# CITlabRostock/citlab-article-separation-new

Measured on AMD Instinct MI355X. Metric: newspaper pages/sec (ARU-Net seg + GNN relation) at 3000x4500 px, higher is better.
Workload: dtype f32s

## Files before the change

citlab-article-separation-new_amd/csrc/aru_engine.hip:

```cpp
#include <algorithm>
#include <cmath>
#include <cstdlib>
#include <memory>

#include "aru_kernels.h"
#include "res8_kernels.h"
#include "res8v_kernels.h"
#include "bf16_kernels.h"
#include "res8w_kernels.h"
#include "res8ws_kernels.h"
#include "level0_plan.h"
#include "convr_kernels.h"
#include "split_kernels.h"
#include "asep_common.h"
#include "aru_pack.h"

using namespace asep;

namespace {

struct Tensor {
    float* p = nullptr;
    int H = 0, W = 0, C = 0;
    bool bf = false;
    size_t count() const { return (size_t)H * W * C; }
    bf16_t* bp() const { return reinterpret_cast<bf16_t*>(p); }
};

struct PackedConv : ConvPlan {
    float* d_w = nullptr;
    float* d_b = nullptr;
    float* d_wino = nullptr;
    float* d_wv = nullptr;
    bf16_t* d_wb = nullptr;
    bf16_t* d_wb8 = nullptr;
    bf16_t* d_ws = nullptr;
    bf16_t* d_ws16 = nullptr;
};

struct DirectConv {
    int k = 0, cout = 0;
    float* d_w = nullptr;
    float* d_b = nullptr;
};

}

struct asep_aru {
    asep_aru_cfg cfg{};
    std::map<std::string, PackedConv> convs;
    struct ResB { int C = 0; bf16_t* d_w = nullptr; float* d_b = nullptr; };
    std::map<std::string, ResB> resb;
    bf16_t* d_r8b_down_w = nullptr;
    float* d_r8b_down_b = nullptr;
    bf16_t* d_r8b_up_w1 = nullptr;
    bf16_t* d_r8f_up_w1 = nullptr;
    bf16_t* d_r8f_down_w1 = nullptr;
    float* d_r8b_down_w1r = nullptr;
    bool use_res32 = true;
    int walk_mode = 1;
    bool use_deconvs = true;
    bool use_convr = true;
    unsigned char* d_zero_trash = nullptr;
    int fused_act = 0;
    bool use_walk = true;
    bf16_t* d_r8b_up_w = nullptr;
    float* d_r8b_up_b = nullptr;
    float* d_r8b_up_b1 = nullptr;
    DirectConv det_first, att_first;
    float* d_r8_down_wr = nullptr;
    float* d_r8_down_br = nullptr;
    float* d_r8_up_w1 = nullptr;
    float* d_r8_up_wr = nullptr;
    float* d_r8_up_br = nullptr;
    float* d_r8_up_b1 = nullptr;
    float* d_r8v_down_wr = nullptr;
    float* d_r8v_up_w1 = nullptr;
    float* d_r8v_up_wr = nullptr;
    bool r8_valu = true;
    bool use_split_walk = true;
    bf16_t* d_r8ws_down_w = nullptr;
    bf16_t* d_r8ws_up_w = nullptr;
    bf16_t* d_r8ws_up_w1 = nullptr;
    bool use_fused8 = true;
    bool fused8_wanted = true;
    bool fused8_var = false;
    float* d_att_head = nullptr;
    bf16_t* d_att_headb = nullptr;
    float* d_logit_w = nullptr;
    float* d_logit_b = nullptr;
    float* d_logit_wd = nullptr;
    float* d_stats = nullptr;
    double* d_sums = nullptr;
    struct Lane {
        hipStream_t s = nullptr;
        bool own_stream = false;
        hipStream_t side = nullptr;
        hipEvent_t ev_fork = nullptr, ev_join = nullptr, ev_begin = nullptr, ev_done = nullptr;
        hipStream_t bside = nullptr;
        hipEvent_t ev_bfork = nullptr, ev_bjoin = nullptr;
        BufferPool pool;
        ~Lane() {
            if (ev_fork) (void)hipEventDestroy(ev_fork);
            if (ev_bfork) (void)hipEventDestroy(ev_bfork);
            if (ev_bjoin) (void)hipEventDestroy(ev_bjoin);
            if (ev_join) (void)hipEventDestroy(ev_join);
            if (ev_begin) (void)hipEventDestroy(ev_begin);
            if (ev_done) (void)hipEventDestroy(ev_done);
            if (side) (void)hipStreamDestroy(side);
            if (bside) (void)hipStreamDestroy(bside);
            if (own_stream && s) (void)hipStreamDestroy(s);
        }
    };
    std::vector<std::unique_ptr<Lane>> lanes;
    Lane* cur = nullptr;
    int last_nl = 0;
    bool lanes_forced = false;
    int num_lanes = 2;
    std::map<std::string, Tensor> endpoints;
    hipStream_t stream = nullptr;
    std::vector<void*> owned;

    struct ProfRec { int kid; double flops, bytes, xflops; hipEvent_t a, b; };
    int num_cus = 256;
    BufferPool host_stage;
    hipStream_t host_stream = nullptr;
    bool use_xcd_sched = true;
    std::map<std::string, const int32_t*> sched_cache;
    bool bf16 = false;
    bool split = false;
    bool use_c12 = true;
    bool fuse_pool = true;
    bool fuse_act = true;
    bool profiling = false;
    bool prof_detail = false;
    bool prof_in_situ = false;
    std::vector<std::string> prof_names;
    std::vector<ProfRec> prof_recs;
    std::vector<hipEvent_t> ev_pool;
    size_t ev_next = 0;

    ~asep_aru() {
        for (void* p : owned)
            if (p) (void)hipFree(p);
// ... 100 lines not shown
    return d;
}

const int32_t* tile_schedule(asep_aru* m, const Res8Args& a, int nblocks, int unit_h) {
    if (!m->use_xcd_sched || nblocks % 8 != 0 || a.total_tiles < 2 * nblocks) return nullptr;
    std::vector<TileDims> probs;
    for (int i = 0; i < a.nprob; ++i) probs.push_back({a.p[i].tiles_x, (a.p[i].H + unit_h - 1) / unit_h, a.p[i].tile_begin});
    return xcd_schedule(m, probs, a.total_tiles);
}

XcdMap oneshot_map(asep_aru* m, int total, int* n_units) {
    XcdMap xm{0, total};
    if (n_units) *n_units = total;
    if (!m->use_xcd_sched || total < 8 * 64) return xm;
    xm.chunk = (total + 7) / 8;
    if (n_units) *n_units = 8 * xm.chunk;
    return xm;
}

typedef std::vector<Tensor> TL;

Tensor new_tensor(asep_aru* m, int H, int W, int C) {
    Tensor t;
    t.H = H; t.W = W; t.C = C;
    t.p = (float*)m->cur->pool.get(t.count() * sizeof(float));
    return t;
}

inline double tbytes(const Tensor& t) { return (double)t.count() * (t.bf ? 2.0 : 4.0); }

std::string dims_of(const TL& l) {
    std::string d;
    for (size_t i = 0; i < l.size() && i < 3; ++i) d += (i ? "+" : "") + std::to_string(l[i].H) + "x" + std::to_string(l[i].W);
    if (l.size() > 3) d += "+..(" + std::to_string(l.size()) + ")";
    return d;
}

#define ASEP_CONV_LAUNCH(KH_, KW_, MT_, C8_, TH_, DB_, BF_, C12_, MB_)                                                   \
    do {                                                                                                                 \
        ps.set_name("conv_mfma_kernel" + targs({ti(KH_), ti(KW_), ti(MT_), tb(C8_), ti(TH_), tb(DB_), tb(BF_), tb(C12_), ti(MB_)})); \
        hipLaunchKernelGGL((conv_mfma_kernel<KH_, KW_, MT_, C8_, TH_, DB_, BF_, C12_, MB_>), grid, dim3(256), 0, s, a);  \
    } while (0)

template <int KH, int KW>
void launch_conv_k(asep_aru* m, const PackedConv& pc, const ConvArgs& a, int total_tiles, double flops, double bytes,
                   const std::string& scope, const TL& in0, bool big_tile) {
    const int mt = pc.c8 ? 1 : (pc.mtiles % 4 == 0 ? 4 : (pc.mtiles % 2 == 0 ? 2 : 1));
    dim3 grid(total_tiles, pc.mtiles / mt);
    ProfScope ps(m, "conv_mfma_kernel", flops, scope + " " + dims_of(in0) + " " + std::to_string(pc.cin) + "->" + std::to_string(pc.cout));
    ps.bytes = bytes;
    hipStream_t s = m->stream;
    const bool res_op = a.p[0].res != nullptr;
    const bool has_res = res_op || KH != 3;
    if constexpr (KW == 4) {
        if (pc.c12) {
            ASEP_CONV_LAUNCH(KH, KW, 1, false, 16, false, false, true, 2);
            return;
        }
    }
    if constexpr (KH == 3) {
        if (pc.c8 && big_tile && !res_op) {
            ASEP_CONV_LAUNCH(3, 3, 1, true, 16, false, false, false, 4);
            return;
        }
    }
    if (pc.c8) ASEP_CONV_LAUNCH(KH, KW, 1, true, CONV_TH, true, false, false, 2);
    else if (mt == 1 && big_tile && !has_res) ASEP_CONV_LAUNCH(3, 3, 1, false, 16, false, false, false, 4);
    else if (mt == 1 && big_tile) ASEP_CONV_LAUNCH(KH, KW, 1, false, 16, false, false, false, 2);
    else if (mt == 4) ASEP_CONV_LAUNCH(KH, KW, 4, false, CONV_TH, true, false, false, 2);
    else if (mt == 2 && !res_op) ASEP_CONV_LAUNCH(KH, KW, 2, false, CONV_TH, true, false, false, 3);
    else if (mt == 2) ASEP_CONV_LAUNCH(KH, KW, 2, false, CONV_TH, true, false, false, 2);
    else ASEP_CONV_LAUNCH(KH, KW, 1, false, CONV_TH, true, false, false, 2);
}

enum PoolKind { POOL_MAX, POOL_AVG_C1, POOL_CHANSUM };
TL run_pool(asep_aru* m, const TL& in, PoolKind kind);

#define ASEP_CONVS_LAUNCH(KH_, KW_, C16_, MT_, TH_, MB_)                                                              \
    do {                                                                                                              \
        ps.set_name("convs_kernel" + targs({ti(KH_), ti(KW_), tb(C16_), ti(MT_), ti(TH_), ti(MB_)}));                 \
        hipLaunchKernelGGL((convs_kernel<KH_, KW_, C16_, MT_, TH_, MB_>), grid, dim3(256), 0, m->stream, a);          \
    } while (0)

TL run_conv_split(asep_aru* m, const PackedConv& pc, const std::string& scope, const TL& in0, const TL* in1, bool relu_in, bool relu_out,
                  const TL* res, TL* pooled, bool keep_full, int act) {
    const bool fuse_pool = pooled && m->fuse_pool;
    TL out;
    if (keep_full || !fuse_pool)
        for (const Tensor& t : in0) out.push_back(new_tensor(m, t.H, t.W, pc.cout));
    if (fuse_pool) {
        pooled->clear();
        for (const Tensor& t : in0) pooled->push_back(new_tensor(m, (t.H + 1) / 2, (t.W + 1) / 2, pc.cout));
    }
    const bool c16 = pc.smode == 1;
    const bool alds = pc.d_ws16 && pc.mtiles == 1;
    const int mt = (pc.mtiles % 4 == 0 && !c16) ? 4 : (pc.mtiles % 2 == 0 ? 2 : 1);
    const int th = (c16 && pc.kh == 3 && mt == 1) ? 16 : 8;
    for (size_t b0 = 0; b0 < in0.size(); b0 += MAXP) {
        const size_t b1 = std::min(in0.size(), b0 + MAXP);
        ConvArgs a{};
        int tiles = 0;
        double flops = 0, bytes = (double)pc.kh * pc.kw * pc.cin * pc.cout * 4.0;
        for (size_t i = b0; i < b1; ++i) {
            ConvProb& p = a.p[i - b0];
            p.in0 = in0[i].p; p.in1 = in1 ? (*in1)[i].p : nullptr; p.res = res ? (*res)[i].p : nullptr;
            p.out = out.empty() ? nullptr : out[i].p;
            p.pool = fuse_pool ? (*pooled)[i].p : nullptr;
            p.H = p.Ho = in0[i].H; p.W = p.Wo = in0[i].W;
            p.tiles_x = (in0[i].W + 31) / 32;
            p.tile_begin = tiles;
            tiles += p.tiles_x * ((in0[i].H + th - 1) / th);
            flops += 2.0 * in0[i].H * in0[i].W * pc.kh * pc.kw * (double)pc.cin * pc.cout;
            bytes += tbytes(in0[i]) + (in1 ? tbytes((*in1)[i]) : 0.0) + (res ? tbytes((*res)[i]) : 0.0) + (out.empty() ? 0.0 : tbytes(out[i])) +
                     (fuse_pool ? tbytes((*pooled)[i]) : 0.0);
        }
        a.nprob = (int)(b1 - b0);
        a.total_tiles = tiles;
        a.c0 = in0[0].C; a.c1 = in1 ? (*in1)[0].C : 0;
        a.wpk = (const f32x4*)(alds ? pc.d_ws16 : pc.d_ws); a.bias = pc.d_b;
        a.cout = pc.cout; a.mtiles = pc.mtiles; a.groups = alds ? pc.cin / 16 : pc.cin / 32;
        a.relu_in = relu_in; a.relu_out = relu_out; a.act = act;
        a.skip_full = fuse_pool && !keep_full;
        int units = tiles;
        a.xm = oneshot_map(m, tiles, &units);
        dim3 grid(units, pc.mtiles / mt);
        TL sub(in0.begin() + b0, in0.begin() + b1);
        ProfScope ps(m, "convs_kernel", flops, scope + " " + dims_of(sub) + " " + std::to_string(pc.cin) + "->" + std::to_string(pc.cout));
        ps.bytes = bytes;
        if (alds) {
            ps.set_name("convs16_kernel<1,8,3,true>");
            hipLaunchKernelGGL((convs16_kernel<1, 8, 3, true>), grid, dim3(256), 0, m->stream, a);
        } else if (pc.kh == 3) {
            if (c16 && th == 16) ASEP_CONVS_LAUNCH(3, 3, true, 1, 16, 2);
            else if (c16 && mt == 2) ASEP_CONVS_LAUNCH(3, 3, true, 2, 8, 3);
            else if (c16) ASEP_CONVS_LAUNCH(3, 3, true, 1, 8, 3);
            else if (mt == 4) ASEP_CONVS_LAUNCH(3, 3, false, 4, 8, 2);
            else if (mt == 2) ASEP_CONVS_LAUNCH(3, 3, false, 2, 8, 2);
            else ASEP_CONVS_LAUNCH(3, 3, false, 1, 8, 2);
        } else {
            if (c16 && mt == 2) ASEP_CONVS_LAUNCH(4, 4, true, 2, 8, 2);
            else if (c16) ASEP_CONVS_LAUNCH(4, 4, true, 1, 8, 2);
            else { set_error("internal: conv %s (4x4, %d input channels) was packed for the split-product kernel", scope.c_str(), pc.cin); throw ArgError(); }
        }
    }
    if (pooled && !fuse_pool) *pooled = run_pool(m, out, POOL_MAX);
    return out;
}


TL run_conv(asep_aru* m, const std::string& scope, const TL& in0, const TL* in1, bool relu_in, bool relu_out,
            const TL* res, TL* pooled = nullptr, bool keep_full = true, int act = 0) {
    auto it = m->convs.find(scope);
    if (it == m->convs.end()) { set_error("internal: conv %s not packed", scope.c_str()); throw ArgError(); }
    const PackedConv& pc = it->second;
    const int cin = in0[0].C + (in1 ? (*in1)[0].C : 0);
    if (cin != pc.cin) {
        set_error("internal: conv %s expects Cin=%d, got %d", scope.c_str(), pc.cin, cin);
        throw ArgError();
    }
    if (!((pc.kh == 3 && pc.kw == 3) || (pc.kh == 4 && pc.kw == 4))) {
        set_error("conv %s: unsupported kernel size %dx%d", scope.c_str(), pc.kh, pc.kw);
        throw ArgError();
    }
    if (pc.d_wv && pc.cout == 1 && m->r8_valu && !in1 && !res && !pooled) {
        TL out1;
        for (const Tensor& t : in0) out1.push_back(new_tensor(m, t.H, t.W, 1));
        for (size_t b0 = 0; b0 < in0.size(); b0 += MAXP) {
            const size_t b1 = std::min(in0.size(), b0 + MAXP);
            ConvArgs a{};
            int tiles = 0;
            double flops = 0, bytes = 0;
            for (size_t i = b0; i < b1; ++i) {
                ConvProb& p = a.p[i - b0];
                p.in0 = in0[i].p; p.out = out1[i].p;
                p.H = p.Ho = in0[i].H; p.W = p.Wo = in0[i].W;
                p.tiles_x = cdiv(in0[i].W, C1O_T);
                p.tile_begin = tiles;
                tiles += p.tiles_x * cdiv(in0[i].H, C1O_T);
                flops += 2.0 * in0[i].H * in0[i].W * 16.0 * pc.cin;
                bytes += tbytes(in0[i]) + tbytes(out1[i]);
            }
            a.nprob = (int)(b1 - b0);
            a.total_tiles = tiles;
            a.c0 = pc.cin; a.cout = 1;
            a.wpk = (const f32x4*)pc.d_wv; a.bias = pc.d_b;
            a.relu_in = relu_in; a.relu_out = relu_out; a.act = act;
            int units = tiles;
            a.xm = oneshot_map(m, tiles, &units);
            ProfScope ps(m, "conv_c1out_kernel", flops, scope);
            ps.bytes = bytes;
            hipLaunchKernelGGL(conv_c1out_kernel, dim3(units), dim3(256), 0, m->stream, a);
        }
        return out1;
    }
    if (m->split && pc.d_ws) return run_conv_split(m, pc, scope, in0, in1, relu_in, relu_out, res, pooled, keep_full, act);
    const bool wino = pc.d_wino && pc.mtiles > 1;
    const int wino_mt = pc.mtiles % 4 == 0 ? 4 : (pc.mtiles % 2 == 0 ? 2 : 1);
    const bool fuse_pool = pooled && m->fuse_pool && pc.cout % 4 == 0 && (!wino || wino_mt <= 2);
    TL out;
    if (keep_full || !fuse_pool)
        for (const Tensor& t : in0) out.push_back(new_tensor(m, t.H, t.W, pc.cout));
    if (fuse_pool) {
        pooled->clear();
        for (const Tensor& t : in0) pooled->push_back(new_tensor(m, cdiv(t.H, 2), cdiv(t.W, 2), pc.cout));
    }
    const bool big_tile = !wino && (!pc.c8 || (pc.kh == 3 && !res)) && (pc.groups == 1 || (pc.groups == 2 && !res && pc.kh == 3)) && pc.mtiles == 1;
    const int th = big_tile ? 16 : CONV_TH;
    for (size_t b0 = 0; b0 < in0.size(); b0 += MAXP) {
        const size_t b1 = std::min(in0.size(), b0 + MAXP);
        ConvArgs a{};
        int tiles = 0;
        double flops = 0, bytes = (double)pc.kh * pc.kw * pc.cin * pc.cout * 4.0;
        for (size_t i = b0; i < b1; ++i) {
            ConvProb& p = a.p[i - b0];
            p.in0 = in0[i].p; p.in1 = in1 ? (*in1)[i].p : nullptr; p.res = res ? (*res)[i].p : nullptr;
            p.out = out.empty() ? nullptr : out[i].p;
            p.pool = fuse_pool ? (*pooled)[i].p : nullptr;
            p.H = p.Ho = in0[i].H; p.W = p.Wo = in0[i].W;
// ... 1346 lines not shown
        }
        reserve_lds({(const void*)res8_down_kernel<false>, (const void*)res8v_down_kernel<0>, (const void*)res8v_down_kernel<1>, (const void*)res8v_down_kernel<2>},
                    R8_DOWN_LDS, "residual");
    }
    if (m->split && !variant && m->d_r8_down_wr) {
        const Res8wsPack p = pack_res8ws(blob, up);
        m->d_r8ws_up_w = m->put_some(p.up_w);
        m->d_r8ws_up_w1 = m->put_some(p.up_w1);
        m->d_r8ws_down_w = m->put_some(p.down_w);
    }
    m->fused_act = (m->bf16 && variant && !cfg->plain_u && cfg->activation != 0 && m->fused8_wanted && m->fuse_act) ? cfg->activation : 0;
    const bool fusedb = m->bf16 && (!variant || m->fused_act);
    if (fusedb && cfg->res_depth == 3 && cfg->feat_root == 8) {
        const Res8bPack p = pack_res8b(blob, up);
        m->d_r8b_down_w = m->put_some(p.down_w);
        m->d_r8b_down_b = m->put_some(p.down_b);
        m->d_r8f_down_w1 = m->put_some(p.f_down_w1);
        m->d_r8b_down_w1r = m->put_some(p.down_w1r);
        m->d_r8b_up_w = m->put_some(p.up_w);
        m->d_r8b_up_b = m->put_some(p.up_b);
        m->d_r8b_up_w1 = m->put_some(p.up_w1);
        m->d_r8b_up_b1 = m->put_some(p.up_b1);
        m->d_r8f_up_w1 = m->put_some(p.f_up_w1);
    }
    if (fusedb && cfg->res_depth == 3)
        for (int l = 0; l < n; ++l) {
            const int f = cfg->feat_root << l;
            if (f != 8 && f != 16 && !(f == 32 && m->use_res32)) continue;
            for (const char* side : {"down", "up"}) {
                if (side[0] == 'u' && l == n - 1) continue;
                const std::string scope = std::string("aru_net/featMapG/unet_") + side + "_" + std::to_string(l);
                const ResbPack p = pack_resb(blob, scope, f);
                if (p.ok) m->resb[scope] = {f, m->put(p.w), m->put(p.b)};
            }
        }
    const Layer logit = find_layer(blob, "aru_net/logit/class");
    if (!has_shape(logit.w, 4, 4, cfg->feat_root, cfg->n_classes)) {
        set_error("weights: aru_net/logit/class/weights must be [4,4,%d,%d]", cfg->feat_root, cfg->n_classes);
        throw PackRefusal{ASEP_ERR_WEIGHTS};
    }
    m->d_logit_w = m->put(logit.w.data);
    m->d_logit_b = m->put(logit.b.data);
    if (cfg->n_classes == 2) m->d_logit_wd = m->put(pack_logit_diff(logit));
}

}

extern "C" {

asep_aru* asep_aru_load(const void* weight_blob, size_t nbytes, const asep_aru_cfg* cfg) {
    ASEP_GUARD_BEGIN
    if (!cfg || !weight_blob) { set_error("asep_aru_load: null argument"); return nullptr; }
    if (cfg->struct_size != (int32_t)sizeof(asep_aru_cfg)) {
        set_error("asep_aru_load: cfg.struct_size is %d, this library's asep_aru_cfg has %zu bytes (ABI version %d): the binding was "
                  "written against another include/asep_hip.h", cfg->struct_size, sizeof(asep_aru_cfg), ASEP_ABI_VERSION);
        return nullptr;
    }
    if (cfg->channels != 1) { set_error("asep_aru_load: only 1-channel input is supported (ARU_v1.py:115)"); return nullptr; }
    if (cfg->compute_dtype < 0 || cfg->compute_dtype > 2) { set_error("asep_aru_load: compute_dtype %d unknown (0 = fp32, 1 = bf16 MFMA, 2 = fp32 with split bf16 products)", cfg->compute_dtype); return nullptr; }
    if (cfg->scale_space_num < 1 || cfg->res_depth < 1) { set_error("asep_aru_load: bad cfg"); return nullptr; }
    if (cfg->activation < 0 || cfg->activation > 2) { set_error("asep_aru_load: activation %d unknown (0 = relu, 1 = elu, 2 = leaky)", cfg->activation); return nullptr; }
    const bool variant = cfg->activation != 0 || cfg->plain_u != 0;
    if (cfg->plain_u && cfg->use_attention) { set_error("asep_aru_load: graph 'U' has no attention branch (ARU_v1.py:92-97)"); return nullptr; }
    std::map<std::string, HostTensor> blob;
    if (!parse_blob(weight_blob, nbytes, blob)) return nullptr;
    warn_ignored_switches();
    std::unique_ptr<asep_aru> m(new asep_aru());
    m->cfg = *cfg;
    m->bf16 = cfg->compute_dtype == 1;
    m->split = cfg->compute_dtype == 2;
    if (const char* e = getenv("ASEP_FUSE_POOL")) m->fuse_pool = atoi(e) != 0;
    if (const char* e = getenv("ASEP_FUSE_ACT")) m->fuse_act = atoi(e) != 0;
    if (const char* e = getenv("ASEP_C12")) m->use_c12 = atoi(e) != 0;
    if (const char* e = getenv("ASEP_FUSED8")) m->use_fused8 = atoi(e) != 0;
    m->fused8_wanted = m->use_fused8;
    if (variant) m->use_fused8 = false;
    if (const char* e = getenv("ASEP_R8_VALU")) m->r8_valu = atoi(e) != 0;
    m->fused8_var = variant && !cfg->plain_u && cfg->activation != 0 && m->fused8_wanted && m->r8_valu && m->fuse_act && !m->bf16;
    if (const char* e = getenv("ASEP_XCD_SCHED")) m->use_xcd_sched = atoi(e) != 0;
    if (const char* e = getenv("ASEP_BF_RES32")) m->use_res32 = atoi(e) != 0;
    if (const char* e = getenv("ASEP_BF_CONVR")) m->use_convr = atoi(e) != 0;
    if (const char* e = getenv("ASEP_SPLIT_DECONV")) m->use_deconvs = atoi(e) != 0;
    if (const char* e = getenv("ASEP_SPLIT_WALK")) m->use_split_walk = atoi(e) != 0;
    if (const char* e = getenv("ASEP_BF_WALK")) { m->walk_mode = atoi(e); m->use_walk = m->walk_mode != 0; }
    if (const char* e = getenv("ASEP_LANES")) { m->num_lanes = std::max(1, std::min(4, atoi(e))); m->lanes_forced = true; }
    for (int l = 0; l < m->num_lanes; ++l) {
        std::unique_ptr<asep_aru::Lane> L(new asep_aru::Lane());
        bool ok = hipStreamCreateWithFlags(&L->side, hipStreamNonBlocking) == hipSuccess &&
                  hipStreamCreateWithFlags(&L->bside, hipStreamNonBlocking) == hipSuccess &&
                  hipEventCreateWithFlags(&L->ev_fork, hipEventDisableTiming) == hipSuccess &&
                  hipEventCreateWithFlags(&L->ev_bfork, hipEventDisableTiming) == hipSuccess &&
                  hipEventCreateWithFlags(&L->ev_bjoin, hipEventDisableTiming) == hipSuccess &&
                  hipEventCreateWithFlags(&L->ev_join, hipEventDisableTiming) == hipSuccess &&
                  hipEventCreateWithFlags(&L->ev_begin, hipEventDisableTiming) == hipSuccess &&
                  hipEventCreateWithFlags(&L->ev_done, hipEventDisableTiming) == hipSuccess;
        if (ok && l > 0) { ok = hipStreamCreateWithFlags(&L->s, hipStreamNonBlocking) == hipSuccess; L->own_stream = ok; }
        if (!ok) { set_error("asep_aru_load: cannot create streams/events for lane %d", l); return nullptr; }
        m->lanes.push_back(std::move(L));
    }
    m->cur = m->lanes[0].get();
    try {
        load_weights(m.get(), blob, variant);
    } catch (const PackRefusal&) {
        return nullptr;
    }
    {
        hipDeviceProp_t prop;
        int dev = 0;
        if (hipGetDevice(&dev) == hipSuccess && hipGetDeviceProperties(&prop, dev) == hipSuccess && prop.multiProcessorCount > 0)
            m->num_cus = prop.multiProcessorCount;
    }
    m->d_stats = m->alloc<float>(2);
    m->d_sums = m->alloc<double>(2);
    m->d_zero_trash = m->alloc<unsigned char>(8192);
    ASEP_HIP_CHECK_THROW(hipMemset(m->d_zero_trash, 0, 8192));
    return m.release();
    ASEP_GUARD_END_PTR
}

void asep_aru_free(asep_aru* m) { delete m; }

static int forward_lanes(asep_aru* m, int n_pages, const float* const* d_imgs, const int32_t* Hs, const int32_t* Ws, float* const* d_outs,
                         uint8_t* const* d_u8, uint8_t* const* d_mask, float threshold, hipStream_t stream) {
    m->endpoints.clear();
    const int by_pages = m->lanes_forced ? n_pages : n_pages / 4;
    const int nl = (m->profiling || n_pages < 2) ? 1 : std::max(1, std::min<int>((int)m->lanes.size(), by_pages));
    asep_aru::Lane& L0 = *m->lanes[0];
    L0.s = stream;
    if (nl != m->last_nl && n_pages > 1) {
        if (m->last_nl != 0)
            for (auto& Lp : m->lanes) Lp->pool.release();
        m->last_nl = nl;
    }
    if (nl == 1) return forward_impl(m, L0, 0, n_pages, d_imgs, Hs, Ws, d_outs, d_u8, d_mask, threshold);
    ASEP_HIP_CHECK(hipEventRecord(L0.ev_begin, stream));
    int page0 = 0;
    for (int l = 0; l < nl; ++l) {
        asep_aru::Lane& L = *m->lanes[l];
        const int cnt = n_pages / nl + (l < n_pages % nl ? 1 : 0);
        if (l > 0) ASEP_HIP_CHECK(hipStreamWaitEvent(L.s, L0.ev_begin, 0));
        int rc = forward_impl(m, L, page0, cnt, d_imgs + page0, Hs + page0, Ws + page0, d_outs + page0, d_u8 ? d_u8 + page0 : nullptr,
                              d_mask ? d_mask + page0 : nullptr, threshold);
        if (rc) return rc;
        if (l > 0) {
            ASEP_HIP_CHECK(hipEventRecord(L.ev_done, L.s));
            ASEP_HIP_CHECK(hipStreamWaitEvent(stream, L.ev_done, 0));
        }
        page0 += cnt;
    }
    m->stream = stream;
    return ASEP_OK;
}

int asep_aru_forward_dev(asep_aru* m, const float* d_img, int H, int W, float* d_out, uint8_t* d_out_u8,
                         uint8_t* d_out_mask, float threshold, void* stream) {
    ASEP_GUARD_BEGIN
    if (!m || !d_img || !d_out || H < 1 || W < 1) { set_error("asep_aru_forward_dev: bad argument"); return ASEP_ERR_ARG; }
    const int32_t h1 = H, w1 = W;
    return forward_lanes(m, 1, &d_img, &h1, &w1, &d_out, d_out_u8 ? &d_out_u8 : nullptr, d_out_mask ? &d_out_mask : nullptr,
                         threshold, (hipStream_t)stream);
    ASEP_GUARD_END
}

int asep_aru_forward_batch_dev(asep_aru* m, int n_pages, const float* const* d_imgs, int H, int W, float* const* d_outs,
                               uint8_t* const* d_out_u8, uint8_t* const* d_out_mask, float threshold, void* stream) {
    ASEP_GUARD_BEGIN
// ... 161 lines not shown
```

citlab-article-separation-new_amd/csrc/asep_common.hip:

```cpp
#include "asep_common.h"
#include <cstdlib>

namespace asep {

static thread_local char g_err[1024] = "";

void set_error(const char* fmt, ...) {
    va_list ap;
    va_start(ap, fmt);
    vsnprintf(g_err, sizeof(g_err), fmt, ap);
    va_end(ap);
}
const char* get_error() { return g_err; }

void warn_ignored_switches() {
    static bool done = false;
    if (done) return;
    done = true;
    static const char* const gone[] = {
        "ASEP_F32_SPLIT", "ASEP_SPLIT_L0", "ASEP_SPLIT_ALDS", "ASEP_SPLIT_TH16", "ASEP_WINOGRAD", "ASEP_WINO_REG", "ASEP_WINO16", "ASEP_BIGTILE",
        "ASEP_BIGTILE2", "ASEP_XCD_ONESHOT", "ASEP_SIDE_STREAM", "ASEP_FUSED8_VAR", "ASEP_BF_TH8", "ASEP_BF_MTB", "ASEP_BF_W8", "ASEP_BF_R8B",
        "ASEP_BF_R8F", "ASEP_CONVS_DBG", "ASEP_R8S_DBG", "ASEP_MAXP24",
#ifndef ASEP_ABLATION
        "ASEP_GNN_BATCH", "ASEP_GNN_LANES",
#endif
    };
    for (const char* name : gone)
        if (getenv(name))
            fprintf(stderr, "libasep_hip: %s is set but is not a switch of this build (ignored; asep_engine_switches() lists what is read)\n", name);
}

bool parse_blob(const void* blob, size_t nbytes, std::map<std::string, HostTensor>& out) {
    const uint8_t* p = (const uint8_t*)blob;
    if (!p || nbytes < 12 || memcmp(p, "ASEPW001", 8) != 0) {
        set_error("weight blob: bad magic (expected ASEPW001)");
        return false;
    }
    uint32_t n;
    memcpy(&n, p + 8, 4);
    size_t off = 12;
    for (uint32_t i = 0; i < n; ++i) {
        if (off + 2 > nbytes) { set_error("weight blob: truncated"); return false; }
        uint16_t nl;
        memcpy(&nl, p + off, 2);
        off += 2;
        if (off + nl + 1 > nbytes) { set_error("weight blob: truncated"); return false; }
        std::string name((const char*)p + off, nl);
        off += nl;
        uint8_t nd = p[off];
        off += 1;
        HostTensor t;
        if (off + 4u * nd > nbytes) { set_error("weight blob: truncated"); return false; }
        for (int d = 0; d < nd; ++d) {
            uint32_t v;
            memcpy(&v, p + off, 4);
            off += 4;
            t.dims.push_back((int)v);
        }
        size_t cnt = t.count();
        if (off + 4 * cnt > nbytes) { set_error("weight blob: truncated in %s", name.c_str()); return false; }
        t.data.resize(cnt);
        memcpy(t.data.data(), p + off, 4 * cnt);
        off += 4 * cnt;
        out[name] = std::move(t);
    }
    if (off != nbytes) { set_error("weight blob: %zu trailing bytes", nbytes - off); return false; }
    return true;
}

void* BufferPool::get(size_t bytes) {
    if (bytes == 0) bytes = 16;
    if (next_ < bufs_.size()) {
        Buf& b = bufs_[next_];
        if (b.n < bytes) {
            if (b.p) (void)hipFree(b.p);
            b.p = nullptr;
            b.n = 0;
            ASEP_HIP_CHECK_THROW(hipMalloc(&b.p, bytes));
            b.n = bytes;
        }
        ++next_;
        return b.p;
    }
    Buf b{nullptr, 0};
    ASEP_HIP_CHECK_THROW(hipMalloc(&b.p, bytes));
    b.n = bytes;
    bufs_.push_back(b);
    ++next_;
    return b.p;
}

void BufferPool::release() {
    for (auto& b : bufs_)
        if (b.p) (void)hipFree(b.p);
    bufs_.clear();
    next_ = 0;
}

size_t BufferPool::total_bytes() const {
    size_t t = 0;
    for (auto& b : bufs_) t += b.n;
    return t;
}

}

extern "C" {
// ... 64 lines not shown
```

citlab-article-separation-new_amd/csrc/split_kernels.h:

```cpp
#pragma once
#include "bf16_kernels.h"
#include "res8_kernels.h"

namespace asep {

__device__ __forceinline__ void split3_pair(float a, float b, unsigned& h, unsigned& m, unsigned& l) {
    h = pack_bf16x2(a, b);
    const f32x2 r = psub(f32x2{a, b}, f32x2{__uint_as_float(h << 16), __uint_as_float(h & 0xffff0000u)});
    m = pack_bf16x2(r.x, r.y);
    const f32x2 q = psub(r, f32x2{__uint_as_float(m << 16), __uint_as_float(m & 0xffff0000u)});
    l = pack_bf16x2(q.x, q.y);
}
__device__ __forceinline__ void split3_x8(f32x4 v0, f32x4 v1, u32x4& h, u32x4& m, u32x4& l) {
    unsigned hh[4], mm[4], ll[4];
    split3_pair(v0.x, v0.y, hh[0], mm[0], ll[0]);
    split3_pair(v0.z, v0.w, hh[1], mm[1], ll[1]);
    split3_pair(v1.x, v1.y, hh[2], mm[2], ll[2]);
    split3_pair(v1.z, v1.w, hh[3], mm[3], ll[3]);
    h = u32x4{hh[0], hh[1], hh[2], hh[3]};
    m = u32x4{mm[0], mm[1], mm[2], mm[3]};
    l = u32x4{ll[0], ll[1], ll[2], ll[3]};
}

template <int KH, int KW, bool C16, int MT, int TH, int MINB>
__global__ __launch_bounds__(256, MINB) void convs_kernel(const ConvArgs a) {
    constexpr int TW = 32, NT = TH * 2 / 4, NH = NT > 4 ? NT / 2 : NT;
    static_assert(NT % 4 == 0, "a wave owns whole row pairs (fused 2x2 pool)");
    constexpr int LH = TH + KH - 1, LW = TW + KW - 1;
    constexpr int PT = (KH - 1) / 2, PL = (KW - 1) / 2;
    constexpr int TAPS = KH * KW;
    constexpr int SUBS = C16 ? 2 : 4;
    constexpr int PLANE = LH * LW * 32, NPL = C16 ? 1 : 2, PART = NPL * PLANE;
    constexpr int CPS = C16 ? (TAPS + 1) / 2 : TAPS;
    constexpr int NU = LH * LW * SUBS, NLOAD = (NU + 255) / 256;
    static_assert(3 * PART <= 65536, "halo tile of the three parts in 64 KB");
    __shared__ __attribute__((aligned(16))) unsigned char lds[3 * PART];

    const int tid = threadIdx.x, lane = tid & 63, wave = tid >> 6;
    const int j = lane & 15, kk = lane >> 4;
    const int bid = sched_tile(a.xm);
    if (bid < 0) return;
    int pi = 0;
    pi = prob_of_tile(a, bid);
    const ConvProb& P = a.p[pi];
    const int tile = bid - P.tile_begin;
    const int ty = tile / P.tiles_x, tx = tile - ty * P.tiles_x;
    const int x0 = tx * TW, y0 = ty * TH, mt0 = blockIdx.y * MT;
    const int H = P.H, W = P.W, cout = a.cout;

    f32x4 acc[MT][NT];
#pragma unroll
    for (int m = 0; m < MT; ++m) {
        const int c = (mt0 + m) * 16 + kk * 4;
        const f32x4 b4 = c < cout ? *reinterpret_cast<const f32x4*>(a.bias + c) : f32x4{0.f, 0.f, 0.f, 0.f};
#pragma unroll
        for (int n = 0; n < NT; ++n) acc[m][n] = b4;
    }
    int nbase[NT];
#pragma unroll
    for (int n = 0; n < NT; ++n) {
        const int id = wave * NT + n;
        nbase[n] = ((id >> 1) * LW + (id & 1) * 16 + j) * 32 + (kk & 1) * 16 + (C16 ? 0 : (kk >> 1) * PLANE);
    }
    if (P.res) {
#pragma unroll
        for (int m = 0; m < MT; ++m) {
            const int c = (mt0 + m) * 16 + kk * 4;
            if (c < cout) {
#pragma unroll
                for (int n = 0; n < NT; ++n) {
                    const int id = wave * NT + n;
                    const int y = min(y0 + (id >> 1), H - 1), x = min(x0 + (id & 1) * 16 + j, W - 1);
                    acc[m][n] += *reinterpret_cast<const f32x4*>(P.res + ((size_t)y * W + x) * cout + c);
                }
            }
        }
    }
    const int nchunks = (C16 ? 1 : a.groups) * CPS;
    const u32x4* __restrict__ wsrc = reinterpret_cast<const u32x4*>(a.wpk) + (size_t)mt0 * 64 + lane;
    const size_t wpart = (size_t)a.mtiles * 64;
    u32x4 af[3][MT], afn[3][MT];
    auto fetch = [&](int q, u32x4 (&dst)[3][MT]) {
        const u32x4* __restrict__ s0 = wsrc + (size_t)q * 3 * wpart;
#pragma unroll
        for (int s = 0; s < 3; ++s)
#pragma unroll
            for (int m = 0; m < MT; ++m) dst[s][m] = s0[s * wpart + m * 64];
    };
    fetch(0, af);

    int spix[NLOAD], slds[NLOAD];
    unsigned stmask = 0;
#pragma unroll
    for (int i = 0; i < NLOAD; ++i) {
        const int u = min(tid + i * 256, NU - 1);
        const int pix = u / SUBS, sub = u - pix * SUBS;
        const int ly = pix / LW, lx = pix - ly * LW;
        const int gy = y0 - PT + ly, gx = x0 - PL + lx;
        spix[i] = min(max(gy, 0), H - 1) * W + min(max(gx, 0), W - 1);
        slds[i] = (sub >> 1) * PLANE + pix * 32 + (sub & 1) * 16;
        stmask |= ((gy >= 0 && gy < H && gx >= 0 && gx < W && tid + i * 256 < NU) ? 1u : 0u) << i;
    }
    const int sub0 = (tid % SUBS) * 8;
    const int cin = a.c0 + a.c1;

    int q = 0;
    const int ngroups = C16 ? 1 : a.groups;
    for (int g = 0; g < ngroups; ++g) {
        {
            const int c = g * 32 + sub0;
            const bool from0 = c < a.c0;
            const float* __restrict__ src = concat_src(P.in0, P.in1, c, a.c0);
            const int cs = from0 ? a.c0 : a.c1;
            const bool second = c + 4 < cin;
            f32x4 st0[NLOAD], st1[NLOAD];
#pragma unroll
            for (int i = 0; i < NLOAD; ++i) {
                const float* p = src + (size_t)spix[i] * cs;
                st0[i] = *reinterpret_cast<const f32x4*>(p);
                st1[i] = second ? *reinterpret_cast<const f32x4*>(p + 4) : f32x4{0.f, 0.f, 0.f, 0.f};
            }
            if (g > 0) __syncthreads();
#pragma unroll
            for (int i = 0; i < NLOAD; ++i) {
                if (i * 256 + 255 < NU || tid + i * 256 < NU) {
                    f32x4 v0 = st0[i], v1 = st1[i];
                    if (!((stmask >> i) & 1u)) v0 = v1 = f32x4{0.f, 0.f, 0.f, 0.f};
                    if (a.relu_in) { v0 = relu4(v0); v1 = relu4(v1); }
                    u32x4 h, mm, l;
                    split3_x8(v0, v1, h, mm, l);
                    *reinterpret_cast<u32x4*>(lds + slds[i]) = h;
                    *reinterpret_cast<u32x4*>(lds + PART + slds[i]) = mm;
                    *reinterpret_cast<u32x4*>(lds + 2 * PART + slds[i]) = l;
                }
            }
            __syncthreads();
        }
        auto chunk = [&](int toff) {
            fetch(min(q + 1, nchunks - 1), afn);
            __builtin_amdgcn_sched_barrier(0);
#pragma unroll
            for (int nh = 0; nh < NT; nh += NH) {
                u32x4 bh[NH], bm[NH], bl[NH];
#pragma unroll
                for (int n = 0; n < NH; ++n) {
                    const unsigned char* p = lds + nbase[nh + n] + toff;
                    bh[n] = *reinterpret_cast<const u32x4*>(p);
                    bm[n] = *reinterpret_cast<const u32x4*>(p + PART);
                    bl[n] = *reinterpret_cast<const u32x4*>(p + 2 * PART);
                }
#pragma unroll
                for (int m = 0; m < MT; ++m)
#pragma unroll
                    for (int n = 0; n < NH; ++n) {
                        f32x4 c = acc[m][nh + n];
                        c = mfma_bf16_k32(af[2][m], bh[n], c);
                        c = mfma_bf16_k32(af[0][m], bl[n], c);
                        c = mfma_bf16_k32(af[1][m], bm[n], c);
                        c = mfma_bf16_k32(af[1][m], bh[n], c);
                        c = mfma_bf16_k32(af[0][m], bm[n], c);
                        c = mfma_bf16_k32(af[0][m], bh[n], c);
                        acc[m][nh + n] = c;
                    }
            }
#pragma unroll
            for (int s = 0; s < 3; ++s)
#pragma unroll
                for (int m = 0; m < MT; ++m) af[s][m] = afn[s][m];
            ++q;
        };
        if constexpr (C16) {
#pragma unroll
            for (int t = 0; t < CPS; ++t) {
                const int ta = 2 * t, tb = 2 * t + 1 < TAPS ? 2 * t + 1 : TAPS - 1;
                const int oa = ((ta / KW) * LW + ta % KW) * 32, ob = ((tb / KW) * LW + tb % KW) * 32;
                chunk((kk >> 1) ? ob : oa);
            }
        } else {
#pragma unroll 1
            for (int ky = 0; ky < KH; ++ky)
#pragma unroll
                for (int kx = 0; kx < KW; ++kx) chunk((ky * LW + kx) * 32);
        }
    }

    const int Wp = (W + 1) >> 1;
#pragma unroll
    for (int m = 0; m < MT; ++m) {
        const int c = (mt0 + m) * 16 + kk * 4;
        const bool cok = c < cout;
#pragma unroll
        for (int n = 0; n < NT; ++n) {
            const int id = wave * NT + n;
            const int y = y0 + (id >> 1), x = x0 + (id & 1) * 16 + j;
            const bool ok = cok && y < H && x < W;
            const size_t p = ((size_t)min(y, H - 1) * W + min(x, W - 1)) * cout + (cok ? c : 0);
            f32x4 v = acc[m][n];
            if (a.relu_out) v = relu4(v);
            else if (a.act) v = act4(v, a.act);
            acc[m][n] = v;
            if (ok && !a.skip_full) *reinterpret_cast<f32x4*>(P.out + p) = v;
        }
        if (P.pool) {
#pragma unroll
            for (int n = 0; n < NT; ++n) {
                if (n & 2) continue;
                const int id = wave * NT + n;
                const int y = y0 + (id >> 1), x = x0 + (id & 1) * 16 + j;
                pool2_store(acc[m][n], acc[m][n + 2], y + 1 < H, x + 1 < W, (j & 1) == 0 && cok && y < H && x < W,
                            P.pool + ((size_t)(y >> 1) * Wp + (x >> 1)) * cout + (cok ? c : 0));
            }
        }
    }
}


template <int MT, int TH, int MINB, bool ALDS>
__global__ __launch_bounds__(256, MINB) void convs16_kernel(const ConvArgs a) {
    constexpr int KH = 3, KW = 3, TW = 32, NT = TH * 2 / 4;
    static_assert(NT == 4, "8 x 32 tiles: a wave owns two rows");
    constexpr int LH = TH + KH - 1, LW = TW + KW - 1, PT = 1, PL = 1, TAPS = 9, CPS = 5;
    constexpr int PART = LH * LW * 32;
    constexpr int NU = LH * LW * 2, NLOAD = (NU + 255) / 256;
    constexpr int ABUF = ALDS ? 3 * MT * 1024 : 0;
    __shared__ __attribute__((aligned(16))) unsigned char lds[3 * PART + 2 * ABUF + 16];
    unsigned char* const albs = lds + 3 * PART;

    const int tid = threadIdx.x, lane = tid & 63, wave = tid >> 6;
    const int j = lane & 15, kk = lane >> 4;
    const int bid = sched_tile(a.xm);
    if (bid < 0) return;
    int pi = 0;
    pi = prob_of_tile(a, bid);
    const ConvProb& P = a.p[pi];
    const int tile = bid - P.tile_begin;
    const int ty = tile / P.tiles_x, tx = tile - ty * P.tiles_x;
    const int x0 = tx * TW, y0 = ty * TH, mt0 = blockIdx.y * MT;
    const int H = P.H, W = P.W, cout = a.cout;

    f32x4 acc[MT][NT];
#pragma unroll
    for (int m = 0; m < MT; ++m) {
        const int c = (mt0 + m) * 16 + kk * 4;
        const f32x4 b4 = c < cout ? *reinterpret_cast<const f32x4*>(a.bias + c) : f32x4{0.f, 0.f, 0.f, 0.f};
#pragma unroll
        for (int n = 0; n < NT; ++n) acc[m][n] = b4;
    }
    int nbase[NT];
#pragma unroll
    for (int n = 0; n < NT; ++n) {
        const int id = wave * NT + n;
        nbase[n] = ((id >> 1) * LW + (id & 1) * 16 + j) * 32 + (kk & 1) * 16;
    }
    if (P.res) {
#pragma unroll
        for (int m = 0; m < MT; ++m) {
            const int c = (mt0 + m) * 16 + kk * 4;
            if (c < cout) {
#pragma unroll
                for (int n = 0; n < NT; ++n) {
                    const int id = wave * NT + n;
                    const int y = min(y0 + (id >> 1), H - 1), x = min(x0 + (id & 1) * 16 + j, W - 1);
                    acc[m][n] += *reinterpret_cast<const f32x4*>(P.res + ((size_t)y * W + x) * cout + c);
                }
            }
// ... 303 lines not shown
```

Baseline: 149.7.

## Pipeline next channel-group input loads behind MFMA work in split conv kernel

Adds a PIPE variant of the split-precision 3x3 conv kernel for non-C16 layers with mt 2 or 4. The global loads for channel group g+1 are issued during the first tap's MFMA chunk and written to LDS after the current group finishes, so memory latency hides behind compute. For MT=4 the weight prefetch is interleaved per m-row instead of held in a full double-buffer, which lowers register pressure. The trade-off is more live registers for the staged input, an extra barrier per group, and less freedom for the scheduler.

Result: no change. 150.2 (median of 4 runs) (+0.3%).

```diff
diff --git a/citlab-article-separation-new_amd/csrc/aru_engine.hip b/citlab-article-separation-new_amd/csrc/aru_engine.hip
--- a/citlab-article-separation-new_amd/csrc/aru_engine.hip
+++ b/citlab-article-separation-new_amd/csrc/aru_engine.hip
@@ -60,6 +60,7 @@
     bool use_res32 = true;
     int walk_mode = 1;
     bool use_deconvs = true;
+    bool use_split_pipe = true;
     bool use_convr = true;
     unsigned char* d_zero_trash = nullptr;
     int fused_act = 0;
@@ -326,6 +327,12 @@
         hipLaunchKernelGGL((convs_kernel<KH_, KW_, C16_, MT_, TH_, MB_>), grid, dim3(256), 0, m->stream, a);          \
     } while (0)
 
+#define ASEP_CONVS_PIPE_LAUNCH(MT_)                                                                                   \
+    do {                                                                                                              \
+        ps.set_name("convs_kernel" + targs({ti(3), ti(3), tb(false), ti(MT_), ti(8), ti(2), tb(true)}));              \
+        hipLaunchKernelGGL((convs_kernel<3, 3, false, MT_, 8, 2, true>), grid, dim3(256), 0, m->stream, a);           \
+    } while (0)
+
 TL run_conv_split(asep_aru* m, const PackedConv& pc, const std::string& scope, const TL& in0, const TL* in1, bool relu_in, bool relu_out,
                   const TL* res, TL* pooled, bool keep_full, int act) {
     const bool fuse_pool = pooled && m->fuse_pool;
@@ -378,6 +385,8 @@
             if (c16 && th == 16) ASEP_CONVS_LAUNCH(3, 3, true, 1, 16, 2);
             else if (c16 && mt == 2) ASEP_CONVS_LAUNCH(3, 3, true, 2, 8, 3);
             else if (c16) ASEP_CONVS_LAUNCH(3, 3, true, 1, 8, 3);
+            else if (mt == 4 && m->use_split_pipe) ASEP_CONVS_PIPE_LAUNCH(4);
+            else if (mt == 2 && m->use_split_pipe) ASEP_CONVS_PIPE_LAUNCH(2);
             else if (mt == 4) ASEP_CONVS_LAUNCH(3, 3, false, 4, 8, 2);
             else if (mt == 2) ASEP_CONVS_LAUNCH(3, 3, false, 2, 8, 2);
             else ASEP_CONVS_LAUNCH(3, 3, false, 1, 8, 2);
@@ -1890,6 +1899,9 @@
     if (const char* e = getenv("ASEP_BF_CONVR")) m->use_convr = atoi(e) != 0;
     if (const char* e = getenv("ASEP_SPLIT_DECONV")) m->use_deconvs = atoi(e) != 0;
     if (const char* e = getenv("ASEP_SPLIT_WALK")) m->use_split_walk = atoi(e) != 0;
+#ifdef ASEP_ABLATION
+    if (const char* e = getenv("ASEP_SPLIT_PIPE")) m->use_split_pipe = atoi(e) != 0;
+#endif
     if (const char* e = getenv("ASEP_BF_WALK")) { m->walk_mode = atoi(e); m->use_walk = m->walk_mode != 0; }
     if (const char* e = getenv("ASEP_LANES")) { m->num_lanes = std::max(1, std::min(4, atoi(e))); m->lanes_forced = true; }
     for (int l = 0; l < m->num_lanes; ++l) {
diff --git a/citlab-article-separation-new_amd/csrc/asep_common.hip b/citlab-article-separation-new_amd/csrc/asep_common.hip
--- a/citlab-article-separation-new_amd/csrc/asep_common.hip
+++ b/citlab-article-separation-new_amd/csrc/asep_common.hip
@@ -22,7 +22,7 @@
         "ASEP_BIGTILE2", "ASEP_XCD_ONESHOT", "ASEP_SIDE_STREAM", "ASEP_FUSED8_VAR", "ASEP_BF_TH8", "ASEP_BF_MTB", "ASEP_BF_W8", "ASEP_BF_R8B",
         "ASEP_BF_R8F", "ASEP_CONVS_DBG", "ASEP_R8S_DBG", "ASEP_MAXP24",
 #ifndef ASEP_ABLATION
-        "ASEP_GNN_BATCH", "ASEP_GNN_LANES",
+        "ASEP_GNN_BATCH", "ASEP_GNN_LANES", "ASEP_SPLIT_PIPE",
 #endif
     };
     for (const char* name : gone)
diff --git a/citlab-article-separation-new_amd/csrc/split_kernels.h b/citlab-article-separation-new_amd/csrc/split_kernels.h
--- a/citlab-article-separation-new_amd/csrc/split_kernels.h
+++ b/citlab-article-separation-new_amd/csrc/split_kernels.h
@@ -22,7 +22,7 @@
     l = u32x4{ll[0], ll[1], ll[2], ll[3]};
 }
 
-template <int KH, int KW, bool C16, int MT, int TH, int MINB>
+template <int KH, int KW, bool C16, int MT, int TH, int MINB, bool PIPE = false>
 __global__ __launch_bounds__(256, MINB) void convs_kernel(const ConvArgs a) {
     constexpr int TW = 32, NT = TH * 2 / 4, NH = NT > 4 ? NT / 2 : NT;
     static_assert(NT % 4 == 0, "a wave owns whole row pairs (fused 2x2 pool)");
@@ -34,6 +34,8 @@
     constexpr int CPS = C16 ? (TAPS + 1) / 2 : TAPS;
     constexpr int NU = LH * LW * SUBS, NLOAD = (NU + 255) / 256;
     static_assert(3 * PART <= 65536, "halo tile of the three parts in 64 KB");
+    static_assert(!PIPE || (!C16 && NT == NH), "the pipelined form: stages of 32 channels, all n-tiles of a wave in registers");
+    constexpr bool AIP = PIPE && MT == 4;
     __shared__ __attribute__((aligned(16))) unsigned char lds[3 * PART];
 
     const int tid = threadIdx.x, lane = tid & 63, wave = tid >> 6;
@@ -79,8 +81,8 @@
     const int nchunks = (C16 ? 1 : a.groups) * CPS;
     const u32x4* __restrict__ wsrc = reinterpret_cast<const u32x4*>(a.wpk) + (size_t)mt0 * 64 + lane;
     const size_t wpart = (size_t)a.mtiles * 64;
-    u32x4 af[3][MT], afn[3][MT];
-    auto fetch = [&](int q, u32x4 (&dst)[3][MT]) {
+    u32x4 af[3][MT], afn[AIP ? 1 : 3][AIP ? 1 : MT];
+    auto fetch = [&](int q, auto& dst) {
         const u32x4* __restrict__ s0 = wsrc + (size_t)q * 3 * wpart;
 #pragma unroll
         for (int s = 0; s < 3; ++s)
@@ -104,40 +106,56 @@
     const int sub0 = (tid % SUBS) * 8;
     const int cin = a.c0 + a.c1;
 
+    f32x4 st0[NLOAD], st1[NLOAD];
+    const int pc0 = PIPE ? __builtin_amdgcn_readfirstlane(a.c0) : 0, pc1 = PIPE ? __builtin_amdgcn_readfirstlane(a.c1) : 0;
+    auto request = [&](int g) {
+        const int c = g * 32 + sub0;
+        const bool from0 = c < a.c0;
+        const float* __restrict__ src = concat_src(P.in0, P.in1, c, a.c0);
+        const int cs = PIPE ? (from0 ? pc0 : pc1) : (from0 ? a.c0 : a.c1);
+        const bool second = PIPE || c + 4 < cin;
+#pragma unroll
+        for (int i = 0; i < NLOAD; ++i) {
+            const float* p = src + (size_t)spix[i] * cs;
+            st0[i] = *reinterpret_cast<const f32x4*>(p);
+            st1[i] = second ? *reinterpret_cast<const f32x4*>(p + 4) : f32x4{0.f, 0.f, 0.f, 0.f};
+        }
+    };
+    auto deposit = [&]() {
+#pragma unroll
+        for (int i = 0; i < NLOAD; ++i) {
+            if (i * 256 + 255 < NU || tid + i * 256 < NU) {
+                f32x4 v0 = st0[i], v1 = st1[i];
+                if (!((stmask >> i) & 1u)) v0 = v1 = f32x4{0.f, 0.f, 0.f, 0.f};
+                if (a.relu_in) { v0 = relu4(v0); v1 = relu4(v1); }
+                u32x4 h, mm, l;
+                split3_x8(v0, v1, h, mm, l);
+                *reinterpret_cast<u32x4*>(lds + slds[i]) = h;
+                *reinterpret_cast<u32x4*>(lds + PART + slds[i]) = mm;
+                *reinterpret_cast<u32x4*>(lds + 2 * PART + slds[i]) = l;
+            }
+        }
+    };
+
     int q = 0;
     const int ngroups = C16 ? 1 : a.groups;
+    if constexpr (PIPE) {
+        request(0);
+        deposit();
+        __syncthreads();
+    }
     for (int g = 0; g < ngroups; ++g) {
-        {
-            const int c = g * 32 + sub0;
-            const bool from0 = c < a.c0;
-            const float* __restrict__ src = concat_src(P.in0, P.in1, c, a.c0);
-            const int cs = from0 ? a.c0 : a.c1;
-            const bool second = c + 4 < cin;
-            f32x4 st0[NLOAD], st1[NLOAD];
-#pragma unroll
-            for (int i = 0; i < NLOAD; ++i) {
-                const float* p = src + (size_t)spix[i] * cs;
-                st0[i] = *reinterpret_cast<const f32x4*>(p);
-                st1[i] = second ? *reinterpret_cast<const f32x4*>(p + 4) : f32x4{0.f, 0.f, 0.f, 0.f};
-            }
+        if constexpr (!PIPE) {
+            request(g);
             if (g > 0) __syncthreads();
-#pragma unroll
-            for (int i = 0; i < NLOAD; ++i) {
-                if (i * 256 + 255 < NU || tid + i * 256 < NU) {
-                    f32x4 v0 = st0[i], v1 = st1[i];
-                    if (!((stmask >> i) & 1u)) v0 = v1 = f32x4{0.f, 0.f, 0.f, 0.f};
-                    if (a.relu_in) { v0 = relu4(v0); v1 = relu4(v1); }
-                    u32x4 h, mm, l;
-                    split3_x8(v0, v1, h, mm, l);
-                    *reinterpret_cast<u32x4*>(lds + slds[i]) = h;
-                    *reinterpret_cast<u32x4*>(lds + PART + slds[i]) = mm;
-                    *reinterpret_cast<u32x4*>(lds + 2 * PART + slds[i]) = l;
-                }
-            }
+            deposit();
             __syncthreads();
         }
-        auto chunk = [&](int toff) {
-            fetch(min(q + 1, nchunks - 1), afn);
+        auto chunk = [&](int toff, bool req) {
+            if constexpr (!AIP) fetch(min(q + 1, nchunks - 1), afn);
+            if constexpr (PIPE) {
+                if (req) request(g + 1);
+            }
             __builtin_amdgcn_sched_barrier(0);
 #pragma unroll
             for (int nh = 0; nh < NT; nh += NH) {
@@ -150,7 +168,7 @@
                     bl[n] = *reinterpret_cast<const u32x4*>(p + 2 * PART);
                 }
 #pragma unroll
-                for (int m = 0; m < MT; ++m)
+                for (int m = 0; m < MT; ++m) {
 #pragma unroll
                     for (int n = 0; n < NH; ++n) {
                         f32x4 c = acc[m][nh + n];
@@ -162,11 +180,20 @@
                         c = mfma_bf16_k32(af[0][m], bh[n], c);
                         acc[m][nh + n] = c;
                     }
-            }
-#pragma unroll
-            for (int s = 0; s < 3; ++s)
-#pragma unroll
-                for (int m = 0; m < MT; ++m) af[s][m] = afn[s][m];
+                    if constexpr (AIP) {
+                        const u32x4* __restrict__ s0 = wsrc + (size_t)min(q + 1, nchunks - 1) * 3 * wpart + m * 64;
+#pragma unroll
+                        for (int s = 0; s < 3; ++s) af[s][m] = s0[s * wpart];
+                        __builtin_amdgcn_sched_barrier(0);
+                    }
+                }
+            }
+            if constexpr (!AIP) {
+#pragma unroll
+                for (int s = 0; s < 3; ++s)
+#pragma unroll
+                    for (int m = 0; m < MT; ++m) af[s][m] = afn[s][m];
+            }
             ++q;
         };
         if constexpr (C16) {
@@ -174,13 +201,34 @@
             for (int t = 0; t < CPS; ++t) {
                 const int ta = 2 * t, tb = 2 * t + 1 < TAPS ? 2 * t + 1 : TAPS - 1;
                 const int oa = ((ta / KW) * LW + ta % KW) * 32, ob = ((tb / KW) * LW + tb % KW) * 32;
-                chunk((kk >> 1) ? ob : oa);
-            }
+                chunk((kk >> 1) ? ob : oa, false);
+            }
+        } else if constexpr (AIP) {
+#pragma unroll 1
+            for (int ky = 0; ky < KH; ++ky)
+#pragma unroll
+                for (int kx = 0; kx < KW; ++kx) chunk((ky * LW + kx) * 32, kx == 0 && ky == 0 && g + 1 < ngroups);
+        } else if constexpr (PIPE) {
+            if (g + 1 < ngroups) chunk(0, true);
+            else chunk(0, false);
+#pragma unroll
+            for (int kx = 1; kx < KW; ++kx) chunk(kx * 32, false);
+#pragma unroll 1
+            for (int ky = 1; ky < KH; ++ky)
+#pragma unroll
+                for (int kx = 0; kx < KW; ++kx) chunk((ky * LW + kx) * 32, false);
         } else {
 #pragma unroll 1
             for (int ky = 0; ky < KH; ++ky)
 #pragma unroll
-                for (int kx = 0; kx < KW; ++kx) chunk((ky * LW + kx) * 32);
+                for (int kx = 0; kx < KW; ++kx) chunk((ky * LW + kx) * 32, false);
+        }
+        if constexpr (PIPE) {
+            if (g + 1 < ngroups) {
+                __syncthreads();
+                deposit();
+                __syncthreads();
+            }
         }
     }
 
```
